# GerHobbelt/ugrep

Hardware: AMD Instinct MI355X
Metric: GB/s scanned + matches/s, 16 GiB synthetic buffer, 1/2/4/8 MI355X (higher is better)
Workload: dtype u8; 1 GPU; 3-literal alternation 'foo|bar|baz' over 16 GiB synthetic ASCII words; config=c2, pattern=foo|bar|baz, bytes_per_gpu=17179869184, total_bytes=17179869184, corpus_kind=1, parallelism=shard1, tables=reference, word=False, dfa_states=9, dfa_row=256, prefilter_ppm=4

## Files before the change

ugrep_amd/csrc/engine.hip:

```cpp
#include <hip/hip_runtime.h>

#include <cstdio>
#include <cstdlib>
#include <cstring>
#include <algorithm>
#include <atomic>
#include <chrono>
#include <condition_variable>
#include <deque>
#include <mutex>
#include <new>
#include <string>
#include <thread>
#include <future>
#include <vector>

#include "../../include/ugpu.h"
#include "plan.hpp"
#include "scan_kernels.hpp"
#include "tables.hpp"

ugpu::Utf8Params utf8_params(const uint8_t* dbuf, uint64_t len)
{
  static std::atomic<int> cached[64];
// ... 154 lines not shown
  static const bool on = std::getenv("UGPU_TRACE") && std::getenv("UGPU_TRACE")[0] == '1';
  return on;
}
#define UGPU_TRACE(...)                  \
  do {                                   \
    if (trace_on()) {                    \
      std::fprintf(stderr, "[ugpu] " __VA_ARGS__); \
      std::fflush(stderr);               \
    }                                    \
  } while (0)

uint64_t env_u64(const char* name, uint64_t dflt)
{
  const char* v = std::getenv(name);
  return v && *v ? std::strtoull(v, nullptr, 0) : dflt;
}

uint32_t acap_lds_n(const ugpu_dfa* d)
{
  if (!d->amode) return 0;
  const size_t n = d->t.ctx_word ? d->t.acap_rows.size() + d->t.states : d->t.acap.size();
  return n <= kSpAcapLds ? (uint32_t)n : 0u;
}

uint32_t fix_rounds_for(const ScanParams& P)
{
  const uint64_t rec = P.tpb * P.unit ? P.tpb * P.unit : 1;
  uint64_t r = env_u64("UGPU_FIX_BUDGET", 256ull << 10) / rec;
  if (r < 4) r = 4;
  if (r > 16) r = 16;
  return (uint32_t)r;
}

int utf8_scan(const uint8_t* dbuf, uint64_t len, bool nul, uint64_t* pos, void* stream);

bool dfa_xc(const ugpu_dfa* d)
{
  const char* env = std::getenv("UGPU_XC");
  return d->t.xc && !d->t.filter && !d->lb && d->t.cap1 != 0 && (!d->d_wtab || d->xcw) && !(env && env[0] == '0');
}

bool dfa_xu(const ugpu_dfa* d)
{
  const char* env = std::getenv("UGPU_XU");
  const bool off = env && env[0] == '0';
  return d->d_xu && (!d->d_wtab || d->wplus) && !off;
}

void fill_tables(ScanParams& P, const ugpu_dfa* d)
{
  P.trans = d->d_trans;
  P.trans32 = d->d_trans32;
  P.xtrans = d->d_xtrans;
  P.xid = d->d_xid;
  P.xid_rows = d->t.xid_rows;
  P.xg = d->d_xg;
  P.xg_sync = d->d_xg_sync;
  P.xg_cls = d->d_xg_sync ? d->d_xg_sync + 256 : nullptr;
  P.xg_stride = 2 * d->t.xg2_pad;
  P.xg_entries = (uint32_t)((d->t.xg2.size() + 7) & ~size_t(7));
  P.cls = d->d_cls;
  P.caps = d->d_caps;
  P.ntrans_pad = d->ntrans_pad;
  P.start = d->t.start;
  P.accb = d->t.accb;
  P.log_row = d->t.log_row;
  P.nstates = d->t.states;
  P.cap1 = d->t.cap1;
  P.wtab = d->d_wtab;
  P.nwtab = d->nwtab;
  P.xc_cls = d->d_cls + 256;
  P.xc_w = d->xcw ? (d->t.xc_w ? 1u : 2u) : 0u;
  P.xu_tab = dfa_xu(d) ? d->d_xu : nullptr;
  P.xu_bm3 = d->d_xu ? reinterpret_cast<const uint32_t*>(d->d_xu + kXuTab) : nullptr;
  P.xu_null = d->t.xu_null;
  P.acap = d->amode ? d->d_acap : nullptr;
  P.ctx_word = d->amode && d->t.ctx_word ? 1u : 0u;
  P.acap_n = (uint32_t)(P.ctx_word ? d->t.acap_rows.size() : d->t.acap.size());
  P.acap_lds = acap_lds_n(d) != 0 && env_u64("UGPU_SP_ACAP_LDS", 1) != 0 ? 1u : 0u;
  P.amap = P.ctx_word ? d->d_acap + d->t.acap_rows.size() : nullptr;
  P.nul = d->nul ? 1u : 0u;
  P.wstart = d->wstart && env_u64("UGPU_WSTART", 1) != 0 ? 1u : 0u;
  P.ft2 = plan_filter2(d->t, d->plan) ? 1u : 0u;
  P.bol0 = 1;
  P.merge_budget = env_u64("UGPU_MERGE_BUDGET", 4096);
  const uint8_t* ft = d->lb ? d->lb_ft : d->t.ft;
  for (int i = 0; i < 5; ++i)
    P.ft[i] = (uint32_t)ft[4 * i] | ((uint32_t)ft[4 * i + 1] << 8) | ((uint32_t)ft[4 * i + 2] << 16) |
              ((uint32_t)ft[4 * i + 3] << 24);
  P.lb_cls = d->lb ? d->d_lbcls : nullptr;
  P.dom = d->d_dom;
  P.look = d->d_look;
  P.dom_all = d->d_dom && d->t.dom_all ? 1u : 0u;
  P.ng_bitmap = d->d_ngram;
  P.ng_n = d->t.ng_n;
  P.ng_log2 = d->t.ng_log2;
  P.ng_tab_lds = d->d_ngram && ngram_tab_lds(d->t.format, d->ntrans_pad, d->nwtab, d->t.ng_log2) ? 1u : 0u;
  if (d->lb) P.wstart = 0;
}

void geometry(ScanParams& P, const uint8_t* dbuf, uint64_t lo, uint64_t hi, uint64_t read_end, int max_rec,
              uint32_t unit, uint32_t per, uint64_t& off)
{
  off = reinterpret_cast<uintptr_t>(dbuf) & 15u;
  P.g = dbuf - off;
  P.lo = lo + off;
  P.hi = hi + off;
  P.rend = read_end + off;
  const uint64_t t0 = P.lo / unit;
  uint64_t t1 = (P.hi + unit - 1) / unit;
  if (t1 <= t0) t1 = t0 + 1;
  const uint64_t nt = t1 - t0;
  uint64_t nrec = nt < (uint64_t)max_rec ? nt : (uint64_t)max_rec;
  if (nrec == 0) nrec = 1;
  const uint64_t min_rec = (nt * unit + kMaxRecBytes - 1) / kMaxRecBytes;
  if (nrec < min_rec) nrec = min_rec < nt ? min_rec : nt;
  const uint64_t tpr = (nt + nrec - 1) / nrec;
  nrec = (nt + tpr - 1) / tpr;
  const uint64_t grid = (nrec + per - 1) / per;
  P.bob = off;
  P.t0 = t0;
  P.t1 = t1;
  P.tpb = tpr;
  P.unit = unit;
  P.grid = (uint32_t)grid;
  P.nrec = (uint32_t)(grid * per);
  P.max_rounds = fix_rounds_for(P);
}

void geometry_for(ScanParams& P, const ugpu_scanner* s, const uint8_t* dbuf, uint64_t lo, uint64_t hi,
                  uint64_t read_end, uint64_t& off, bool xi = false)
{
  if (s->word)
    geometry(P, dbuf, lo, hi, read_end, s->word_rec, wfind_unit(), s->ngram ? ngram_waves() : wfind_waves(), off);
  else if (xi && s->xc)
    geometry(P, dbuf, lo, hi, read_end, s->xi_rec, xc_unit(s->xu), xc_waves(), off);
  else if (xi && s->xg)
    geometry(P, dbuf, lo, hi, read_end, s->xi_rec, xg_unit(), xg_waves(), off);
  else if (xi)
    geometry(P, dbuf, lo, hi, read_end, s->xi_rec, xi_unit(), xi_waves(), off);
  else if (s->sparse)
    geometry(P, dbuf, lo, hi, read_end, s->max_rec, kWaveTile, kSpWaves, off);
  else
    geometry(P, dbuf, lo, hi, read_end, s->max_rec, dense_unit(s->dfa->t.format), dense_waves(s->dfa->t.format), off);
}

hipError_t launch_main(const ugpu_scanner* s, const ScanParams& P, bool write, hipStream_t st, bool xi = false)
{
  if (s->word && s->ngram) return launch_ngram(P, s->dfa->t.format, write, st);
  if (s->word) return launch_wfind(P, s->dfa->t.format, write, st);
  if (xi && s->xc) return launch_xc(P, write, st);
  if (xi && s->xg) return launch_xg(P, st);
  if (xi) return launch_xi(P, s->xi_smem, st);
  if (s->sparse) return launch_sparse(P, write, s->smem, st);
  return launch_dense(P, s->dfa->t.format, write, s->smem, st);
}

bool is_device_ptr(const void* p)
{
  hipPointerAttribute_t a;
  if (hipPointerGetAttributes(&a, p) != hipSuccess) {
    (void)hipGetLastError();
    return false;
  }
  return a.type == hipMemoryTypeDevice;
}
// ... 2803 lines not shown
```

ugrep_amd/csrc/scan_kernels.hpp:

```cpp
#pragma once
#include <hip/hip_runtime.h>
#include <cstdint>

namespace ugpu {

constexpr int kMaxRec = 8192;
constexpr int kFixThreads = 1024;
constexpr int kWaveTile = 4096;
constexpr int kSpWaves = 4;
#ifndef UGPU_DSEG_BYTE
#define UGPU_DSEG_BYTE 188
#endif
#ifndef UGPU_DSEG_CLASS
#define UGPU_DSEG_CLASS 92
#endif
#ifndef UGPU_DWAVES_BYTE
#define UGPU_DWAVES_BYTE 4
#endif
#ifndef UGPU_DWAVES_CLASS
#define UGPU_DWAVES_CLASS 8
#endif
constexpr int kDSegByte = UGPU_DSEG_BYTE;
constexpr int kDSegClass = UGPU_DSEG_CLASS;
constexpr int kDWavesByte = UGPU_DWAVES_BYTE;
// ... 36 lines not shown
};
constexpr uint64_t kOpenConvBudget = 4096;
constexpr uint64_t kOpenSlack = 256;

struct DevTotals {
  uint64_t count, digest, dcap, entry, exit;
  uint32_t flags, rounds;
};

#define UGPU_FLAG_HALO 1u
#define UGPU_FLAG_CAPACITY 2u
#define UGPU_FLAG_BUDGET 4u
#define UGPU_FLAG_WSLOW 32u
#define UGPU_FLAG_NEEDWRITE 64u
#define UGPU_FLAG_USLOW 128u
#define UGPU_FLAG_UMIX 256u
#define UGPU_FLAG_OPEN 512u
constexpr uint32_t kStageOver = 0xffffffffu;
constexpr uint32_t kStageDone = 0xfffffffeu;
constexpr uint32_t kStagePer = 1024;

struct ScanParams {
  const uint8_t* g;
  uint64_t lo, hi;
  uint64_t rend;
  int64_t delta;
  uint32_t at_eof;
  uint32_t ablate;
  uint32_t zero;
  uint64_t t0, t1, tpb;
  uint32_t unit;
  uint32_t nrec;
  uint32_t nstates;
  const uint16_t* trans;
  const uint16_t* xtrans;
  const uint8_t* xid;
  uint32_t xid_rows;
  const uint16_t* xg;
  const uint8_t* xg_sync;
  const uint8_t* xg_cls;
  uint32_t xg_stride;
  uint32_t xg_entries;
  const uint8_t* cls;
  const uint32_t* trans32;
  const uint32_t* caps;
  uint32_t ntrans_pad;
  uint32_t start, accb, log_row;
  uint32_t ft[5];
  uint32_t cap1;
  uint32_t grid;
  BlockRec* recs;
  const uint64_t* entries;
  const uint64_t* out_base;
  uint64_t* out_start;
  uint32_t* out_len;
  uint32_t* out_cap;
  uint64_t out_capacity;
  uint64_t* out_fix;
  uint32_t* flags;
  DevTotals* totals;
  uint64_t* entries_out;
  uint64_t* out_base_out;
  const uint32_t* wtab;
  uint32_t nwtab;
  uint64_t bob;
  uint32_t max_rounds;
  uint64_t merge_budget;
  const uint8_t* xc_cls;
  uint64_t* st_start;
  uint32_t* st_len;
  uint32_t* st_cap;
  uint32_t* st_n;
  uint32_t st_per;
  uint32_t xc_w;
  uint32_t xu_w;
  uint32_t xu_exact;
  const uint8_t* xu_tab;
  const uint32_t* xu_bm3;
  uint32_t xu_null;
  uint16_t* inbits;
  const uint32_t* acap;
  uint32_t wstart;
  uint32_t ft2;
  const uint32_t* lb_cls;
  const uint32_t* dom;
  const uint32_t* look;
  uint32_t dom_all;
  uint32_t bol0;
  uint32_t nul;
  uint32_t ctx_word;
  uint32_t acap_n;
  const uint32_t* amap;
  uint32_t acap_lds;
  OpenRec* open;
  uint32_t* susp;
  SuspRec* srec;
  const uint32_t* ng_bitmap;
  uint32_t ng_n, ng_log2, ng_tab_lds;
};

struct ForestArgs {
  uint64_t c_lo, c_hi;
  uint32_t nblk;
  uint32_t* ex;
  uint64_t* entry;
  uint64_t* run;
  uint64_t* bentry;
  uint64_t* bsum;
  uint64_t* bbase;
};
constexpr uint64_t kFChunk = 64ull << 20;
hipError_t launch_forest(const ScanParams& P, uint32_t format, const ForestArgs& A, uint64_t entry, bool write,
                         DevTotals* tot, hipStream_t stream);
uint64_t forest_block();

hipError_t launch_fix(const ScanParams& P, uint32_t format, hipStream_t stream);
hipError_t launch_pack_records(const uint64_t* start, const uint32_t* len, const uint32_t* cap, uint64_t n,
                               uint64_t base, uint8_t* out, int caps, int dense, uint64_t* esc, uint32_t* nesc,
                               hipStream_t stream);
hipError_t launch_chain_fix(const ScanParams& P, uint32_t format, uint64_t old_entry, uint64_t new_entry,
                            hipStream_t stream);
hipError_t launch_gen(int kind, uint64_t seed, uint64_t off, uint8_t* dbuf, uint64_t len, hipStream_t stream);
hipError_t launch_sparse(const ScanParams& P, bool write, size_t smem, hipStream_t stream);
hipError_t launch_stage_copy(const ScanParams& P, hipStream_t stream);
hipError_t sparse_occupancy(const ScanParams& P, size_t smem, int* blocks_per_cu);
size_t sparse_smem_bytes(uint32_t ntrans_pad, uint32_t nstates, uint32_t nlds_acap = 0);
constexpr uint32_t kSpAcapLds = 2048;
struct LineRec {
  uint64_t first_line, last_line;
  uint64_t trans;
  uint64_t nmatch;
};
struct LinesParams {
  const uint8_t* g;
  uint64_t len;
  uint64_t per;
  uint64_t nwaves;
  const uint64_t* starts;
  uint64_t nmatch;
  uint64_t* counts;
  const uint64_t* prefix;
  uint64_t* lines;
  LineRec* recs;
  uint16_t* qcount;
};
hipError_t launch_nl_count(const LinesParams& L, bool sparse, hipStream_t stream);
hipError_t launch_nl_assign(const LinesParams& L, bool sparse, hipStream_t stream);
uint32_t lines_tile();
constexpr uint32_t kLinesQuarter = 1024;
struct SelParams {
  const uint8_t* g;
  uint64_t len;
  uint64_t per;
  uint64_t nwaves;
  const uint64_t* starts;
  const uint32_t* lens;
  uint64_t nmatch;
  uint32_t invert;
  uint64_t* lastnl;
  uint64_t* mcover;
  const uint64_t* prefix;
  const uint64_t* bol;
  const uint64_t* cover;
  const uint64_t* obase;
  uint64_t* selcnt;
  uint64_t* begin;
// ... 83 lines not shown
```

ugrep_amd/csrc/sparse_kernel.hip:

```cpp
#include "device_common.hpp"

#ifndef UGPU_SP_CTX_OCC
#define UGPU_SP_CTX_OCC 4
#endif
#ifndef UGPU_SP_CTX_WIN
#define UGPU_SP_CTX_WIN 1
#endif

namespace ugpu {

namespace {

struct FTab {
  uint32_t t0lo, t0hi, t1lo, t1hi, t2;
};

template <bool FT2>
__device__ __forceinline__ uint32_t bucket_bits(uint32_t x, const FTab& F)
{
  const uint32_t r0 = __builtin_amdgcn_perm(F.t0hi, F.t0lo, x & 0x07070707u);
  const uint32_t r1 = __builtin_amdgcn_perm(F.t1hi, F.t1lo, (x >> 3) & 0x07070707u);
  if constexpr (FT2) return r0 & r1;
  const uint32_t r2 = __builtin_amdgcn_perm(F.t2, F.t2, (x >> 6) & 0x03030303u);
  return r0 & r1 & r2;
}

__device__ __forceinline__ uint32_t cand_flags(uint32_t R, uint32_t Rn)
{
  return R & __builtin_amdgcn_alignbit(Rn, R, 10) & __builtin_amdgcn_alignbit(Rn, R, 20);
}

__device__ __forceinline__ uint32_t flags4(uint32_t X)
{
  return ((((X | (X >> 1)) & 0x01010101u) * 0x01020408u) >> 24);
}

__device__ __forceinline__ uint32_t letters4(uint32_t x)
{
  const uint32_t t = (x | 0x20202020u) & 0x7f7f7f7fu;
  const uint32_t m = (t + 0x1f1f1f1fu) & ~(t + 0x05050505u) & ~x & 0x80808080u;
  return ((m >> 7) * 0x01020408u) >> 24;
}

__device__ __forceinline__ uint32_t letters16(const uint4& v)
{
  return letters4(v.x) | (letters4(v.y) << 4) | (letters4(v.z) << 8) | (letters4(v.w) << 12);
}

__device__ __forceinline__ uint32_t dpp_scan_add(uint32_t v)
{
  v += __builtin_amdgcn_update_dpp(0, v, 0x111, 0xf, 0xf, false);
  v += __builtin_amdgcn_update_dpp(0, v, 0x112, 0xf, 0xf, false);
  v += __builtin_amdgcn_update_dpp(0, v, 0x114, 0xf, 0xf, false);
  v += __builtin_amdgcn_update_dpp(0, v, 0x118, 0xf, 0xf, false);
  v += __builtin_amdgcn_update_dpp(0, v, 0x142, 0xa, 0xf, false);
  v += __builtin_amdgcn_update_dpp(0, v, 0x143, 0xc, 0xf, false);
  return v;
}

__device__ __forceinline__ uint32_t umax32(uint32_t a, uint32_t b) { return a > b ? a : b; }

__device__ __forceinline__ uint32_t dpp_scan_max(uint32_t v)
{
  v = umax32(v, __builtin_amdgcn_update_dpp(0, v, 0x111, 0xf, 0xf, false));
  v = umax32(v, __builtin_amdgcn_update_dpp(0, v, 0x112, 0xf, 0xf, false));
  v = umax32(v, __builtin_amdgcn_update_dpp(0, v, 0x114, 0xf, 0xf, false));
  v = umax32(v, __builtin_amdgcn_update_dpp(0, v, 0x118, 0xf, 0xf, false));
  v = umax32(v, __builtin_amdgcn_update_dpp(0, v, 0x142, 0xa, 0xf, false));
  v = umax32(v, __builtin_amdgcn_update_dpp(0, v, 0x143, 0xc, 0xf, false));
  return v;
}

__device__ __forceinline__ uint32_t dpp_prev_lane(uint32_t v) { return __builtin_amdgcn_update_dpp(0, v, 0x138, 0xf, 0xf, false); }

__device__ __forceinline__ uint4 load16(const uint8_t* g, uint64_t pos, uint64_t last16)
{
  return *reinterpret_cast<const uint4*>(g + (pos < last16 ? pos : last16));
}

struct TileLoad {
  __amdgpu_buffer_rsrc_t rs;
};

__device__ __forceinline__ uint4 stream16(const TileLoad& L, uint32_t off)
{
  typedef unsigned int v4u __attribute__((ext_vector_type(4)));
  const v4u v = __builtin_amdgcn_raw_buffer_load_b128(L.rs, (int)off, 0, 2 );
  return uint4{v.x, v.y, v.z, v.w};
}

__device__ __forceinline__ void wave_lds_sync()
{
  __builtin_amdgcn_fence(__ATOMIC_RELEASE, "wavefront");
  __builtin_amdgcn_wave_barrier();
  __builtin_amdgcn_fence(__ATOMIC_ACQUIRE, "wavefront");
}

__device__ __forceinline__ uint32_t lanes_below(uint64_t ballot)
{
  return __builtin_amdgcn_mbcnt_hi((uint32_t)(ballot >> 32), __builtin_amdgcn_mbcnt_lo((uint32_t)ballot, 0u));
}

constexpr int kDefer = 64;
constexpr int kAux = 2048;
static_assert(kDefer * 8 <= kAux && 64 * 32 <= kAux, "aux region too small");

struct Stage {
  uint64_t* start = nullptr;
  uint32_t* len = nullptr;
  uint32_t* cap = nullptr;
  uint64_t n = 0;
  uint32_t over = 0;
};

struct WaveChain {
  uint64_t x;
  uint32_t dn;
  uint64_t widx;
  uint32_t wover;
  uint32_t ovf;
  CountEm acc;
  Stage sg;
  uint32_t first, open;
  uint64_t c1, e1;
  uint32_t le1;
  uint32_t pend;
  uint64_t rs, ptile;
  uint64_t wlo;
  uint64_t lbr, lbs;
  uint64_t whi;
};

__device__ __forceinline__ uint64_t readlane64(uint64_t v, int l)
{
  const uint32_t hi = (uint32_t)__builtin_amdgcn_readlane((uint32_t)(v >> 32), l);
  const uint32_t lo = (uint32_t)__builtin_amdgcn_readlane((uint32_t)v, l);
  return ((uint64_t)hi << 32) | lo;
}

template <bool WRITE, bool STAGE = false>
__device__ __forceinline__ void resolve(bool valid, uint64_t c, uint64_t len, uint32_t le, int lane, const Ctx& C,
                                        const ScanParams& P, WaveChain& w)
{
  const uint64_t x = w.x;
  const bool vm = valid && len != 0 && c >= x;
  const uint64_t endr = vm ? c + len - x : 0;
  const bool wide = __ballot(endr > 0xffffffffull) != 0;
  const uint32_t er = (uint32_t)endr, cr = vm ? (uint32_t)(c - x) : 0u;
  const uint32_t pm = dpp_prev_lane(dpp_scan_max(er));
  bool kept = vm && cr >= pm;
  if (wide || __ballot(vm && cr < pm)) {
    uint64_t xx = x;
    kept = false;
    const uint64_t e = vm ? c + len : 0ull;
#pragma unroll 1
    for (int i = 0; i < 64; ++i) {
      const uint64_t ci = __shfl(c, i, 64), ei = __shfl(e, i, 64);
      if (ei != 0 && ci >= xx) {
        if (lane == i) kept = true;
        xx = ei;
      }
    }
  }
  const uint64_t kb = __ballot(kept);
  if (!kb) return;
  const uint64_t rb = __ballot(kept && C.caps[le >> C.log_row] != kCapRedo);
  if constexpr (WRITE) {
    WriteEm we{w.widx + lanes_below(rb), P.out_capacity, P.out_start, P.out_len, P.out_cap};
    if (kept) we.put(C, c, len, le, +1);
    w.wover |= we.overflow;
    w.widx += __popcll(rb);
  } else {
    if (kept) w.acc.put(C, c, len, le, +1);
    if constexpr (STAGE) {
      WriteEm se{w.sg.n + lanes_below(rb), P.st_per, w.sg.start, w.sg.len, w.sg.cap};
      if (kept) se.put(C, c, len, le, +1);
      w.sg.over |= se.overflow;
      w.sg.n += __popcll(rb);
    }
    if (!w.first) {
      const int f = __builtin_ctzll(kb);
      w.first = 1;
      w.c1 = readlane64(c, f);
      w.e1 = w.c1 + readlane64(len, f);
      w.le1 = (uint32_t)__builtin_amdgcn_readlane(le, f);
    }
  }
  w.x = readlane64(c + len, 63 - __builtin_clzll(kb));
// ... 175 lines not shown
    if (s2 > w.x) w.x = s2;
  }
}

template <bool WRITE, bool STAGE>
__device__ __forceinline__ void batch_finish(BatchLane& L, int lane, uint8_t* scr, const Tab<0>& T, const Ctx& C,
                                             const ScanParams& P, WaveChain& w, uint64_t lim, uint64_t gw)
{
  for (;;) {
    const int i = batch_resolve<WRITE, STAGE>(L, lane, C, P, w);
    if (i == 64) break;
    long_lane<WRITE, STAGE>(i, L, lane, scr, T, C, P, w, lim, gw);
    if (w.x == kOpenEnd) break;
  }
  wave_lds_sync();
}

constexpr uint64_t kLbStart = 1ull << 63;
__device__ __forceinline__ bool lb_in(const ScanParams& P, uint32_t b) { return (P.lb_cls[b >> 5] >> (b & 31)) & 1u; }

__device__ __forceinline__ uint64_t lb_back_wave(const ScanParams& P, uint64_t pl, uint64_t bl, int lane)
{
  while (pl > bl) {
    const bool inr = (uint64_t)lane < pl - bl;
    const uint32_t b = inr ? (uint32_t)P.g[pl - 1 - lane] : 0u;
    const uint64_t stop = __ballot(inr && !lb_in(P, b));
    if (stop) return pl - (uint64_t)__builtin_ctzll(stop);
    if (pl - bl <= 64) return bl;
    pl -= 64;
  }
  return pl;
}

__device__ __forceinline__ uint64_t lb_batch(const ScanParams& P, uint64_t e, bool listed, int lane, uint32_t dn,
                                             WaveChain& w)
{
  const bool fixed = listed && (e >> 63) != 0;
  const uint64_t n = listed ? (e & ~kLbStart) : w.lbr;
  const uint32_t plo = (uint32_t)__shfl_up((int)(uint32_t)n, 1, 64);
  const uint32_t phi = (uint32_t)__shfl_up((int)(uint32_t)(n >> 32), 1, 64);
  uint64_t bound = lane == 0 ? w.lbr : (((uint64_t)phi << 32) | plo);
  if (bound < w.wlo) bound = w.wlo;
  if (bound > n) bound = n;
  uint64_t p = n;
  uint32_t steps = 0;
  if (listed && !fixed)
    while (p > bound && steps < 64 && lb_in(P, P.g[p - 1])) {
      --p;
      ++steps;
    }
  const bool longl = listed && !fixed && p > bound && lb_in(P, P.g[p - 1]);
  for (uint64_t lm = __ballot(longl); lm; lm &= lm - 1) {
    const int L = __builtin_ctzll(lm);
    const uint64_t r = lb_back_wave(P, readlane64(p, L), readlane64(bound, L), lane);
    if (lane == L) p = r;
  }
  const bool found = fixed || (listed && p > bound) || (listed && p == bound && bound == w.wlo);
  uint64_t st = found ? p : 0;
#pragma unroll
  for (int d = 1; d < 64; d <<= 1) {
    const uint32_t lo2 = (uint32_t)__shfl_up((int)(uint32_t)st, d, 64);
    const uint32_t hi2 = (uint32_t)__shfl_up((int)(uint32_t)(st >> 32), d, 64);
    const uint64_t o = ((uint64_t)hi2 << 32) | lo2;
    if (lane >= d && o > st) st = o;
  }
  if (w.lbs > st) st = w.lbs;
  const int last = (int)dn - 1;
  w.lbr = readlane64(n, last);
  w.lbs = readlane64(st, last);
  return st;
}

template <bool WRITE, int ABL, int W = kWalkPlain, bool STAGE = false, bool RESUME = false, bool LB = false>
__device__ __forceinline__ void flush_deferred(const uint64_t* dl, uint8_t* scr, uint32_t dn, int lane, const Tab<0>& T,
                                            const Ctx& C, const ScanParams& P, WaveChain& w, uint64_t lim,
                                            uint64_t gw)
{
  wave_lds_sync();
  const bool listed = (uint32_t)lane < dn;
  const uint64_t craw = listed ? dl[lane] : 0;
  bool valid = listed;
  uint64_t c = craw;
  if constexpr (LB) c = lb_batch(P, craw, listed, lane, dn, w);
  const uint64_t a = c & ~uint64_t(15);
  if constexpr (W != kWalkCtx || UGPU_SP_CTX_WIN) {
    const uint64_t last16 = (P.rend - 1) & ~uint64_t(15);
    const uint4 v0 = load16(P.g, a, last16), v1 = load16(P.g, a + 16, last16);
    wave_lds_sync();
    *reinterpret_cast<uint4*>(scr + 32 * lane) = v0;
    *reinterpret_cast<uint4*>(scr + 32 * lane + 16) = v1;
  }
  wave_lds_sync();
  if constexpr (W != kWalkPlain) {
    uint64_t len = 0;
    uint32_t le = 0;
    if (valid && ABL != 3) {
      Win win = win_of(P);
      if constexpr (W == kWalkCtx) {
        if (P.acap_lds) {
          win.acap = C.caps;
          win.amap = C.caps + P.acap_n;
        }
      }
      if constexpr (W == kWalkWord || UGPU_SP_CTX_WIN) {
        win.wl = scr + 32 * lane;
        win.wa = a;
        win.wn = 32;
      }
      len = walk<0, W>(T, win, c, le, w.ovf);
    }
    resolve<WRITE, STAGE>(valid, c, len, le, lane, C, P, w);
    wave_lds_sync();
    return;
  }
  BatchLane L{c, T.start, 0u, 0u, 0u, 0u, valid};
  if (valid && ABL != 3) {
    const uint64_t wl = a + 32 < lim ? a + 32 : lim;
    const uint32_t wr = (uint32_t)(wl - c);
    for (;;) {
      if (L.qr >= wr) {
        if (c + L.qr >= P.rend) {
          if (!P.at_eof) w.ovf = 1;
        } else {
          L.st = c + L.qr >= lim ? 2u : 1u;
        }
        break;
      }
      const uint32_t e = T.step(L.s, scr[32 * lane + (uint32_t)(c - a) + L.qr]);
      if (e == 0) break;
      L.s = e;
      ++L.qr;
      if (e >= T.accb) {
        L.lr = L.qr;
        L.le = e;
      }
    }
  }
  if (!__ballot(L.st != 0)) {
    resolve<WRITE, STAGE>(valid, c, L.lr, L.le, lane, C, P, w);
    wave_lds_sync();
    return;
  }
  wave_lds_sync();
  if constexpr (RESUME) {
    batch_finish<WRITE, STAGE>(L, lane, scr, T, C, P, w, lim, gw);
  } else {
    PendSlot ps;
    ps.c = L.c;
    ps.s = L.s;
    ps.le = L.le;
    ps.packed = L.qr | L.lr << 8 | L.st << 16 | (uint32_t)L.todo << 24;
    ps.pad = 0;
    P.srec[gw].lanes[lane] = ps;
    w.pend = 1;
    w.rs = readlane64(LB ? craw & ~kLbStart : craw, (int)dn - 1) + 1;
  }
}

template <bool WRITE, int ABL, int W = kWalkPlain, bool STAGE = false, bool RESUME = false, bool LB = false,
          bool FT2 = false>
__device__ __forceinline__ void tile_pass(const uint4& v0, const uint4& v1, const uint4& v2, const uint4& v3,
                                          uint64_t ts, bool edge, uint64_t wlo, uint64_t whi, int lane,
                                          const FTab& F, const Tab<0>& T, const Ctx& C, const ScanParams& P,
                                          uint64_t* dl, uint8_t* scr, WaveChain& w, uint64_t lim, uint64_t gw)
{
  if constexpr (ABL == 1) {
    w.acc.cnt += (v0.x ^ v1.y ^ v2.z ^ v3.w) & 1;
    return;
  }
  if (!RESUME && w.pend) return;
  const uint32_t h0 = bucket_bits<FT2>(v0.x, F), h1 = bucket_bits<FT2>(v1.x, F), h2 = bucket_bits<FT2>(v2.x, F),
                 h3 = bucket_bits<FT2>(v3.x, F);
  const uint32_t n0 = __builtin_amdgcn_update_dpp(0, h0, 0x130, 0xf, 0xf, false);
  const uint32_t n1 = __builtin_amdgcn_update_dpp(0, h1, 0x130, 0xf, 0xf, false);
  const uint32_t n2 = __builtin_amdgcn_update_dpp(0, h2, 0x130, 0xf, 0xf, false);
  const uint32_t n3 = __builtin_amdgcn_update_dpp(0, h3, 0x130, 0xf, 0xf, false);
  const uint32_t s1 = __builtin_amdgcn_readlane(h1, 0), s2 = __builtin_amdgcn_readlane(h2, 0),
                 s3 = __builtin_amdgcn_readlane(h3, 0);
  const bool l63 = lane == 63;
  const uint32_t e0 = l63 ? s1 : n0, e1 = l63 ? s2 : n1, e2 = l63 ? s3 : n2, e3 = l63 ? 0x3f3f3f3fu : n3;
  uint32_t X[4][4];
  {
    const uint32_t y = bucket_bits<FT2>(v0.y, F), z = bucket_bits<FT2>(v0.z, F), u = bucket_bits<FT2>(v0.w, F);
    X[0][0] = cand_flags(h0, y);
    X[0][1] = cand_flags(y, z);
    X[0][2] = cand_flags(z, u);
    X[0][3] = cand_flags(u, e0);
  }
  {
    const uint32_t y = bucket_bits<FT2>(v1.y, F), z = bucket_bits<FT2>(v1.z, F), u = bucket_bits<FT2>(v1.w, F);
    X[1][0] = cand_flags(h1, y);
    X[1][1] = cand_flags(y, z);
    X[1][2] = cand_flags(z, u);
    X[1][3] = cand_flags(u, e1);
  }
  {
    const uint32_t y = bucket_bits<FT2>(v2.y, F), z = bucket_bits<FT2>(v2.z, F), u = bucket_bits<FT2>(v2.w, F);
    X[2][0] = cand_flags(h2, y);
    X[2][1] = cand_flags(y, z);
    X[2][2] = cand_flags(z, u);
    X[2][3] = cand_flags(u, e2);
  }
  {
    const uint32_t y = bucket_bits<FT2>(v3.y, F), z = bucket_bits<FT2>(v3.z, F), u = bucket_bits<FT2>(v3.w, F);
    X[3][0] = cand_flags(h3, y);
    X[3][1] = cand_flags(y, z);
    X[3][2] = cand_flags(z, u);
    X[3][3] = cand_flags(u, e3);
  }
  uint32_t lt01 = 0, lt23 = 0;
  if (P.wstart) {
    lt01 = letters16(v0) | (letters16(v1) << 16);
    lt23 = letters16(v2) | (letters16(v3) << 16);
  }
  const uint32_t any0 = X[0][0] | X[0][1] | X[0][2] | X[0][3], any1 = X[1][0] | X[1][1] | X[1][2] | X[1][3];
  const uint32_t any2 = X[2][0] | X[2][1] | X[2][2] | X[2][3], any3 = X[3][0] | X[3][1] | X[3][2] | X[3][3];
  const bool tail = !P.at_eof && ts + kWaveTile + 2 > P.rend && ts < P.rend;
  if (!tail && !__ballot((any0 | any1 | any2 | any3) != 0)) return;
  const uint32_t anyk[4] = {any0, any1, any2, any3};
#pragma unroll
  for (int k = 0; k < 4; ++k) {
    if (!tail && !__ballot(anyk[k] != 0)) continue;
    uint32_t mk = flags4(X[k][0]) | (flags4(X[k][1]) << 4) | (flags4(X[k][2]) << 8) | (flags4(X[k][3]) << 12);
    if (P.wstart) mk &= ~(((k < 2 ? lt01 : lt23) >> (16 * (k & 1))) << 1) & 0xffffu;
    const uint64_t p0 = ts + 1024u * k + 16u * lane;
    if (!P.at_eof && p0 + 18 > P.rend && p0 < P.rend) {
      const uint64_t lo2 = P.rend >= 2 ? P.rend - 2 : 0;
      const uint64_t a = lo2 > p0 ? lo2 - p0 : 0, z = P.rend - p0 > 16 ? 16 : P.rend - p0;
      mk |= (uint32_t)((lowbits(z) & ~lowbits(a)) & 0xffffu);
    }
    if (edge) {
      const uint64_t a = wlo > p0 ? (wlo - p0 > 16 ? 16 : wlo - p0) : 0;
      const uint64_t z = whi > p0 ? (whi - p0 > 16 ? 16 : whi - p0) : 0;
      mk &= (uint32_t)((lowbits(z) & ~lowbits(a)) & 0xffffu);
    }
    const uint64_t xr = w.x > w.rs ? w.x : w.rs;
    if (xr > p0) {
      const uint64_t a = xr - p0;
      mk &= (uint32_t)(~lowbits(a < 16 ? a : 16) & 0xffffu);
    }
    if constexpr (ABL == 2) {
      w.acc.cnt += __popc(mk);
      continue;
    }
    const uint32_t cnt = __popc(mk);
    const uint32_t incl = dpp_scan_add(cnt);
    const uint32_t tot = (uint32_t)__builtin_amdgcn_readlane(incl, 63);
    const uint32_t rank = incl - cnt;
    for (uint32_t done = 0; done < tot;) {
      if (w.dn == (uint32_t)kDefer) {
        flush_deferred<WRITE, ABL, W, STAGE, RESUME, LB>(dl, scr, w.dn, lane, T, C, P, w, lim, gw);
        w.dn = 0;
        if (!RESUME && w.pend) {
          w.ptile = ts;
          return;
        }
      }
      const uint32_t take = tot - done < kDefer - w.dn ? tot - done : kDefer - w.dn;
      uint32_t m = mk, r = rank;
      while (m) {
        const uint32_t bit = __builtin_ctz(m);
        m &= m - 1;
        if (r - done < take) dl[w.dn + r - done] = p0 + bit;
        ++r;
      }
      w.dn += take;
      done += take;
    }
  }
}

__device__ __forceinline__ TileLoad wave_tile(const uint8_t* wbase, uint32_t i, uint32_t rel)
{
  const uint32_t off = i * (uint32_t)kWaveTile;
  const uint32_t n = rel > off ? rel - off : 0u;
  const int nr = __builtin_amdgcn_readfirstlane((int)(n < (uint32_t)kWaveTile ? n : (uint32_t)kWaveTile));
  return TileLoad{__builtin_amdgcn_make_buffer_rsrc(const_cast<uint8_t*>(wbase + off), (short)0, nr, 0x00020000)};
}

}

template <bool WRITE, int ABL, int W = kWalkPlain, bool STAGE = false, bool RESUME = false, bool LB = false,
          bool FT2 = false>
__global__ __launch_bounds__(kSpWaves * 64, RESUME ? 1 : (W == kWalkCtx ? UGPU_SP_CTX_OCC : 6)) void sparse_kernel(ScanParams P)
{
  extern __shared__ __attribute__((aligned(16))) uint8_t smem[];
  const int tid = threadIdx.x, lane = tid & 63;
  const int wid = __builtin_amdgcn_readfirstlane(tid >> 6);
  const uint64_t gw = (uint64_t)blockIdx.x * kSpWaves + wid;
  bool mine = true;
  if constexpr (RESUME) {
    mine = P.susp[gw] != 0;
    if (!__syncthreads_or(mine)) return;
  }
  uint8_t* aux = smem + wid * kAux;
  uint64_t* dl = reinterpret_cast<uint64_t*>(aux);
  uint8_t* scr = aux;
  uint16_t* ltrans = reinterpret_cast<uint16_t*>(smem + kSpWaves * kAux);
  uint32_t* lcaps = reinterpret_cast<uint32_t*>(ltrans + P.ntrans_pad);
  {
    const uint4* src = reinterpret_cast<const uint4*>(P.trans);
    uint4* dst = reinterpret_cast<uint4*>(ltrans);
    for (uint32_t i = tid; i < P.ntrans_pad / 8; i += kSpWaves * 64) dst[i] = src[i];
    for (uint32_t i = tid; i < P.nstates; i += kSpWaves * 64) lcaps[i] = P.caps[i];
    if constexpr (W == kWalkCtx) {
      if (P.acap_lds) {
        uint32_t* la = lcaps + P.nstates;
        for (uint32_t i = tid; i < P.acap_n; i += kSpWaves * 64) la[i] = P.acap[i];
        if (P.ctx_word)
          for (uint32_t i = tid; i < P.nstates; i += kSpWaves * 64) la[P.acap_n + i] = P.amap[i];
      }
    }
  }
  __syncthreads();
  if (!mine) return;
  const Tab<0> T{ltrans, nullptr, P.start, P.accb};
  const Ctx C = W == kWalkCtx ? Ctx{P.acap_lds ? lcaps + P.nstates : P.acap, 0u, P.delta}
                              : Ctx{lcaps, P.log_row, P.delta};
  const FTab F{P.ft[0], P.ft[1], P.ft[2], P.ft[3], P.ft[4]};

  uint64_t tb = P.t0 + gw * P.tpb;
  uint64_t te = tb + P.tpb < P.t1 ? tb + P.tpb : P.t1;
  if (tb > te) tb = te;
  const uint64_t wlo = clampu(tb * kWaveTile, P.lo, P.hi);
  const uint64_t whi = clampu(te * kWaveTile, P.lo, P.hi);
  WaveChain w;
  w.x = WRITE ? P.entries[gw] : wlo;
  w.dn = 0;
  w.widx = WRITE ? P.out_base[gw] : 0;
  w.wover = 0;
  w.ovf = 0;
  w.first = w.open = 0;
  w.c1 = w.e1 = 0;
  w.le1 = 0;
  w.pend = 0;
  w.rs = w.ptile = 0;
  w.wlo = wlo;
  w.whi = whi;
  w.lbr = w.lbs = wlo;
  const uint64_t lim = (W == kWalkPlain && P.open && whi < P.hi) ? whi : P.rend;
  if constexpr (WRITE && !RESUME) {
    if (P.st_n && P.st_n[gw] == kStageDone) {
      if (P.susp && lane == 0) P.susp[gw] = 0;
      return;
    }
  }
  if constexpr (STAGE) {
    w.sg.start = P.st_start + gw * P.st_per;
    w.sg.len = P.st_len + gw * P.st_per;
    w.sg.cap = P.st_cap + gw * P.st_per;
  }

  const uint32_t n = (uint32_t)(te - tb);
  const uint8_t* wbase = P.g + tb * kWaveTile;
  const uint64_t rend16 = (P.rend + 15) & ~uint64_t(15), wb = tb * kWaveTile;
  const uint64_t relw = rend16 > wb ? rend16 - wb : 0;
  const uint32_t rel = (uint32_t)(relw < (uint64_t)n * kWaveTile ? relw : (uint64_t)n * kWaveTile);
  const bool clip_lo = wlo != wb, clip_hi = whi != te * kWaveTile;
  const uint32_t lo16 = 16u * lane;
  uint32_t i = 0;
  if constexpr (RESUME) {
    const SuspRec& sr = P.srec[gw];
    w.x = sr.x;
    w.widx = sr.widx;
    w.wover = sr.wover;
    w.ovf = sr.ovf;
    w.acc.cnt = lane == 0 ? sr.cnt : 0;
    w.acc.dg = lane == 0 ? sr.dg : 0;
    w.acc.dc = lane == 0 ? sr.dc : 0;
    w.sg.n = sr.sgn;
    w.sg.over = sr.sgover;
    w.first = sr.first;
    w.open = sr.open;
    w.c1 = sr.c1;
    w.e1 = sr.e1;
    w.le1 = sr.le1;
    w.rs = sr.rs;
    w.lbr = sr.lbr;
    w.lbs = sr.lbs;
    i = sr.tile;
    const PendSlot ps = sr.lanes[lane];
    BatchLane L{ps.c, ps.s, ps.packed & 0xffu, (ps.packed >> 8) & 0xffu, ps.le, (ps.packed >> 16) & 0xffu,
                (ps.packed >> 24) != 0};
    batch_finish<WRITE, STAGE>(L, lane, scr, T, C, P, w, lim, gw);
  }
  if constexpr (!RESUME && W != kWalkCtx) {
    if (LB && whi > wlo && lb_in(P, P.g[wlo])) {
      if (lane == 0) dl[0] = wlo | kLbStart;
      wave_lds_sync();
      w.dn = 1;
    }
  }
  uint4 a0, a1, a2, a3, b0, b1, b2, b3;
  {
    const TileLoad La = wave_tile(wbase, i, rel);
    a0 = stream16(La, lo16);
    a1 = stream16(La, lo16 + 1024);
    a2 = stream16(La, lo16 + 2048);
    a3 = stream16(La, lo16 + 3072);
    const TileLoad Lb = wave_tile(wbase, i + 1, rel);
    b0 = stream16(Lb, lo16);
    b1 = stream16(Lb, lo16 + 1024);
    b2 = stream16(Lb, lo16 + 2048);
    b3 = stream16(Lb, lo16 + 3072);
  }
  if (n >= i + 2) {
    do {
      tile_pass<WRITE, ABL, W, STAGE, RESUME, LB, FT2>(a0, a1, a2, a3, wb + (uint64_t)i * kWaveTile, i == 0 && clip_lo,
                                                       wlo, whi, lane, F, T, C, P, dl, scr, w, lim, gw);
      {
        const TileLoad L = wave_tile(wbase, i + 2, rel);
        a0 = stream16(L, lo16);
        a1 = stream16(L, lo16 + 1024);
        a2 = stream16(L, lo16 + 2048);
        a3 = stream16(L, lo16 + 3072);
      }
      tile_pass<WRITE, ABL, W, STAGE, RESUME, LB, FT2>(b0, b1, b2, b3, wb + (uint64_t)(i + 1) * kWaveTile,
                                                       i + 2 == n && clip_hi, wlo, whi, lane, F, T, C, P, dl, scr, w,
                                                       lim, gw);
      {
        const TileLoad L = wave_tile(wbase, i + 3, rel);
        b0 = stream16(L, lo16);
        b1 = stream16(L, lo16 + 1024);
        b2 = stream16(L, lo16 + 2048);
        b3 = stream16(L, lo16 + 3072);
      }
      i += 2;
    } while (i + 1 < n);
  }
  if (i < n)
    tile_pass<WRITE, ABL, W, STAGE, RESUME, LB, FT2>(a0, a1, a2, a3, wb + (uint64_t)i * kWaveTile,
                                                     (i == 0 && clip_lo) || clip_hi, wlo, whi, lane, F, T, C, P, dl,
                                                     scr, w, lim, gw);
  if constexpr (LB) {
    if (!w.pend && whi > wlo && lb_in(P, P.g[whi - 1])) {
      const uint64_t r = lb_back_wave(P, whi, wlo, lane);
      {
        if (w.dn == (uint32_t)kDefer) {
          w.ptile = te * kWaveTile;
          flush_deferred<WRITE, ABL, W, STAGE, RESUME, LB>(dl, scr, w.dn, lane, T, C, P, w, lim, gw);
          w.dn = 0;
        }
        if (!w.pend) {
          wave_lds_sync();
          if (lane == 0) dl[w.dn] = r | kLbStart;
          wave_lds_sync();
          ++w.dn;
        }
      }
    }
  }
  if (!w.pend && w.dn) {
    flush_deferred<WRITE, ABL, W, STAGE, RESUME, LB>(dl, scr, w.dn, lane, T, C, P, w, lim, gw);
    w.ptile = te * kWaveTile;
  }
  if constexpr (!RESUME) {
    if (P.susp) {
      if (w.pend) {
        const uint64_t c = wave_sum(w.acc.cnt), d = wave_sum(w.acc.dg), dc = wave_sum(w.acc.dc);
        if (lane == 0) {
          SuspRec* sr = P.srec + gw;
          sr->x = w.x;
          sr->widx = w.widx;
          sr->cnt = c;
          sr->dg = d;
          sr->dc = dc;
          sr->c1 = w.c1;
          sr->e1 = w.e1;
          sr->rs = w.rs;
          sr->lbr = w.lbr;
          sr->lbs = w.lbs;
          sr->sgn = w.sg.n;
          sr->wover = w.wover;
          sr->ovf = w.ovf;
          sr->first = w.first;
          sr->open = w.open;
          sr->le1 = w.le1;
          sr->sgover = w.sg.over;
          sr->tile = (uint32_t)((w.ptile - wb) / kWaveTile);
          sr->dn = 0;
          P.susp[gw] = 1;
        }
        return;
      }
      if (lane == 0) P.susp[gw] = 0;
    }
  }
  uint64_t x = w.x > whi ? w.x : whi;
  if (tb == te) x = wlo;
  if (w.open) x = lim;

  if (w.ovf) atomicOr(P.flags, UGPU_FLAG_HALO);
  if (!WRITE && w.open && lane == 0) atomicOr(P.flags, UGPU_FLAG_OPEN);
  if (w.wover) atomicOr(P.flags, UGPU_FLAG_CAPACITY);
  if constexpr (!WRITE) {
    const uint64_t c = wave_sum(w.acc.cnt), d = wave_sum(w.acc.dg), dc = wave_sum(w.acc.dc);
    if (STAGE && lane == 0) P.st_n[gw] = w.sg.over ? kStageOver : (uint32_t)w.sg.n;
    if (lane == 0) {
      BlockRec rec;
      rec.entry = wlo;
      rec.exit = x;
      rec.cnt = c;
      rec.dg = d;
      rec.dc = dc;
      rec.pad0 = rec.pad1 = rec.pad2 = 0;
      if (W == kWalkPlain) {
        rec.pad0 = w.c1;
        rec.pad1 = w.first ? w.e1 : 0;
// ... 127 lines not shown
```

Before: 6413 GB/s.

## Capture candidate byte windows from registers during sparse scan to skip global reloads

For the plain, non-line-buffered walk, the sparse tile pass now stores each candidate's 32-byte window into a per-slot LDS area straight from the tile registers, taking the next lane's bytes through DPP and readlane. The deferred batch then reloads from global memory only for candidates flagged global, such as the lane-63 edge of the last chunk. It also packs candidate flags with v_lshl_or, uses a ballot-based rank when each lane has at most one candidate, and enlarges the per-wave aux LDS region. The aim is to remove scattered global reloads and a wave sync per deferred batch, at the cost of extra LDS per wave (lower occupancy risk) and more register shuffling on candidate tiles.

```diff
diff --git a/ugrep_amd/csrc/engine.hip b/ugrep_amd/csrc/engine.hip
--- a/ugrep_amd/csrc/engine.hip
+++ b/ugrep_amd/csrc/engine.hip
@@ -260,6 +260,7 @@
   P.nul = d->nul ? 1u : 0u;
   P.wstart = d->wstart && env_u64("UGPU_WSTART", 1) != 0 ? 1u : 0u;
   P.ft2 = plan_filter2(d->t, d->plan) ? 1u : 0u;
+  P.sp_win = env_u64("UGPU_SP_WIN", 1) != 0 ? 1u : 0u;
   P.bol0 = 1;
   P.merge_budget = env_u64("UGPU_MERGE_BUDGET", 4096);
   const uint8_t* ft = d->lb ? d->lb_ft : d->t.ft;
diff --git a/ugrep_amd/csrc/scan_kernels.hpp b/ugrep_amd/csrc/scan_kernels.hpp
--- a/ugrep_amd/csrc/scan_kernels.hpp
+++ b/ugrep_amd/csrc/scan_kernels.hpp
@@ -142,6 +142,7 @@
   const uint32_t* acap;
   uint32_t wstart;
   uint32_t ft2;
+  uint32_t sp_win;
   const uint32_t* lb_cls;
   const uint32_t* dom;
   const uint32_t* look;
diff --git a/ugrep_amd/csrc/sparse_kernel.hip b/ugrep_amd/csrc/sparse_kernel.hip
--- a/ugrep_amd/csrc/sparse_kernel.hip
+++ b/ugrep_amd/csrc/sparse_kernel.hip
@@ -28,6 +28,14 @@
 __device__ __forceinline__ uint32_t cand_flags(uint32_t R, uint32_t Rn)
 {
   return R & __builtin_amdgcn_alignbit(Rn, R, 10) & __builtin_amdgcn_alignbit(Rn, R, 20);
+}
+
+__device__ __forceinline__ uint32_t pack_flags(const uint32_t (&X)[4])
+{
+  const uint32_t lo = X[0] | (X[1] << 2), hi = X[2] | (X[3] << 2);
+  uint32_t r;
+  asm("v_lshl_or_b32 %0, %1, 4, %2" : "=v"(r) : "v"(hi), "v"(lo));
+  return r;
 }
 
 __device__ __forceinline__ uint32_t flags4(uint32_t X)
@@ -102,8 +110,12 @@
 }
 
 constexpr int kDefer = 64;
-constexpr int kAux = 2048;
-static_assert(kDefer * 8 <= kAux && 64 * 32 <= kAux, "aux region too small");
+constexpr int kList = kDefer * 8;
+constexpr int kAux = kList + kDefer * 32;
+static_assert(kAux % 16 == 0 && kList % 16 == 0 && 64 * 16 <= kDefer * 32, "aux region layout");
+constexpr uint64_t kWinGlobal = 1ull << 62;
+template <int W, bool LB>
+constexpr bool capture_windows = W == kWalkPlain && !LB;
 
 struct Stage {
   uint64_t* start = nullptr;
@@ -445,15 +457,27 @@
   bool valid = listed;
   uint64_t c = craw;
   if constexpr (LB) c = lb_batch(P, craw, listed, lane, dn, w);
+  if constexpr (capture_windows<W, LB>) c = craw & ~kWinGlobal;
   const uint64_t a = c & ~uint64_t(15);
-  if constexpr (W != kWalkCtx || UGPU_SP_CTX_WIN) {
+  if constexpr (capture_windows<W, LB>) {
+    const bool glob = listed && (craw & kWinGlobal) != 0;
+    if (__ballot(glob)) {
+      if (glob) {
+        const uint64_t last16 = (P.rend - 1) & ~uint64_t(15);
+        const uint4 v0 = load16(P.g, a, last16), v1 = load16(P.g, a + 16, last16);
+        *reinterpret_cast<uint4*>(scr + 32 * lane) = v0;
+        *reinterpret_cast<uint4*>(scr + 32 * lane + 16) = v1;
+      }
+      wave_lds_sync();
+    }
+  } else if constexpr (W != kWalkCtx || UGPU_SP_CTX_WIN) {
     const uint64_t last16 = (P.rend - 1) & ~uint64_t(15);
     const uint4 v0 = load16(P.g, a, last16), v1 = load16(P.g, a + 16, last16);
     wave_lds_sync();
     *reinterpret_cast<uint4*>(scr + 32 * lane) = v0;
     *reinterpret_cast<uint4*>(scr + 32 * lane + 16) = v1;
   }
-  wave_lds_sync();
+  if constexpr (!capture_windows<W, LB>) wave_lds_sync();
   if constexpr (W != kWalkPlain) {
     uint64_t len = 0;
     uint32_t le = 0;
@@ -516,7 +540,7 @@
     ps.pad = 0;
     P.srec[gw].lanes[lane] = ps;
     w.pend = 1;
-    w.rs = readlane64(LB ? craw & ~kLbStart : craw, (int)dn - 1) + 1;
+    w.rs = readlane64(LB ? craw & ~kLbStart : c, (int)dn - 1) + 1;
   }
 }
 
@@ -572,22 +596,41 @@
     X[3][3] = cand_flags(u, e3);
   }
   uint32_t lt01 = 0, lt23 = 0;
-  if (P.wstart) {
+  if (!capture_windows<W, LB> && P.wstart) {
     lt01 = letters16(v0) | (letters16(v1) << 16);
     lt23 = letters16(v2) | (letters16(v3) << 16);
   }
-  const uint32_t any0 = X[0][0] | X[0][1] | X[0][2] | X[0][3], any1 = X[1][0] | X[1][1] | X[1][2] | X[1][3];
-  const uint32_t any2 = X[2][0] | X[2][1] | X[2][2] | X[2][3], any3 = X[3][0] | X[3][1] | X[3][2] | X[3][3];
+  constexpr bool CAP = capture_windows<W, LB>;
+  uint32_t any0, any1, any2, any3;
+  if constexpr (CAP) {
+    any0 = pack_flags(X[0]);
+    any1 = pack_flags(X[1]);
+    any2 = pack_flags(X[2]);
+    any3 = pack_flags(X[3]);
+  } else {
+    any0 = X[0][0] | X[0][1] | X[0][2] | X[0][3], any1 = X[1][0] | X[1][1] | X[1][2] | X[1][3];
+    any2 = X[2][0] | X[2][1] | X[2][2] | X[2][3], any3 = X[3][0] | X[3][1] | X[3][2] | X[3][3];
+  }
   const bool tail = !P.at_eof && ts + kWaveTile + 2 > P.rend && ts < P.rend;
   if (!tail && !__ballot((any0 | any1 | any2 | any3) != 0)) return;
   const uint32_t anyk[4] = {any0, any1, any2, any3};
 #pragma unroll
   for (int k = 0; k < 4; ++k) {
     if (!tail && !__ballot(anyk[k] != 0)) continue;
-    uint32_t mk = flags4(X[k][0]) | (flags4(X[k][1]) << 4) | (flags4(X[k][2]) << 8) | (flags4(X[k][3]) << 12);
-    if (P.wstart) mk &= ~(((k < 2 ? lt01 : lt23) >> (16 * (k & 1))) << 1) & 0xffffu;
+    uint32_t mk;
+    if constexpr (CAP)
+      mk = flags4(anyk[k]) | (flags4(anyk[k] >> 2) << 4) | (flags4(anyk[k] >> 4) << 8) |
+           (flags4(anyk[k] >> 6) << 12);
+    else
+      mk = flags4(X[k][0]) | (flags4(X[k][1]) << 4) | (flags4(X[k][2]) << 8) | (flags4(X[k][3]) << 12);
+    if constexpr (CAP) {
+      if (P.wstart) mk &= ~(letters16(k == 0 ? v0 : k == 1 ? v1 : k == 2 ? v2 : v3) << 1) & 0xffffu;
+    } else {
+      if (P.wstart) mk &= ~(((k < 2 ? lt01 : lt23) >> (16 * (k & 1))) << 1) & 0xffffu;
+    }
+    const uint64_t cs = ts + 1024u * k;
     const uint64_t p0 = ts + 1024u * k + 16u * lane;
-    if (!P.at_eof && p0 + 18 > P.rend && p0 < P.rend) {
+    if ((CAP ? tail : !P.at_eof) && p0 + 18 > P.rend && p0 < P.rend) {
       const uint64_t lo2 = P.rend >= 2 ? P.rend - 2 : 0;
       const uint64_t a = lo2 > p0 ? lo2 - p0 : 0, z = P.rend - p0 > 16 ? 16 : P.rend - p0;
       mk |= (uint32_t)((lowbits(z) & ~lowbits(a)) & 0xffffu);
@@ -598,7 +641,7 @@
       mk &= (uint32_t)((lowbits(z) & ~lowbits(a)) & 0xffffu);
     }
     const uint64_t xr = w.x > w.rs ? w.x : w.rs;
-    if (xr > p0) {
+    if ((!CAP || xr > cs) && xr > p0) {
       const uint64_t a = xr - p0;
       mk &= (uint32_t)(~lowbits(a < 16 ? a : 16) & 0xffffu);
     }
@@ -607,9 +650,16 @@
       continue;
     }
     const uint32_t cnt = __popc(mk);
-    const uint32_t incl = dpp_scan_add(cnt);
-    const uint32_t tot = (uint32_t)__builtin_amdgcn_readlane(incl, 63);
-    const uint32_t rank = incl - cnt;
+    uint32_t rank, tot;
+    if (CAP && !__ballot(cnt > 1)) {
+      const uint64_t hb = __ballot(mk != 0);
+      rank = lanes_below(hb);
+      tot = (uint32_t)__popcll(hb);
+    } else {
+      const uint32_t incl = dpp_scan_add(cnt);
+      tot = (uint32_t)__builtin_amdgcn_readlane(incl, 63);
+      rank = incl - cnt;
+    }
     for (uint32_t done = 0; done < tot;) {
       if (w.dn == (uint32_t)kDefer) {
         flush_deferred<WRITE, ABL, W, STAGE, RESUME, LB>(dl, scr, w.dn, lane, T, C, P, w, lim, gw);
@@ -620,17 +670,54 @@
         }
       }
       const uint32_t take = tot - done < kDefer - w.dn ? tot - done : kDefer - w.dn;
+      const uint4& vc = k == 0 ? v0 : k == 1 ? v1 : k == 2 ? v2 : v3;
+      uint4 nx{0u, 0u, 0u, 0u};
+      bool glob = false;
+      if constexpr (CAP) {
+        glob = !P.sp_win || (k == 3 && l63);
+        if (P.sp_win) {
+          nx.x = __builtin_amdgcn_update_dpp(0, vc.x, 0x130, 0xf, 0xf, false);
+          nx.y = __builtin_amdgcn_update_dpp(0, vc.y, 0x130, 0xf, 0xf, false);
+          nx.z = __builtin_amdgcn_update_dpp(0, vc.z, 0x130, 0xf, 0xf, false);
+          nx.w = __builtin_amdgcn_update_dpp(0, vc.w, 0x130, 0xf, 0xf, false);
+          if (k < 3) {
+            const uint4& vn = k == 0 ? v1 : k == 1 ? v2 : v3;
+            const uint32_t sx = __builtin_amdgcn_readlane(vn.x, 0), sy = __builtin_amdgcn_readlane(vn.y, 0),
+                           sz = __builtin_amdgcn_readlane(vn.z, 0), sw = __builtin_amdgcn_readlane(vn.w, 0);
+            if (l63) nx = uint4{sx, sy, sz, sw};
+          }
+        }
+      }
       uint32_t m = mk, r = rank;
       while (m) {
         const uint32_t bit = __builtin_ctz(m);
         m &= m - 1;
-        if (r - done < take) dl[w.dn + r - done] = p0 + bit;
+        if (r - done < take) {
+          const uint32_t slot = w.dn + r - done;
+          dl[slot] = CAP ? (p0 + bit) | (glob ? kWinGlobal : 0ull) : p0 + bit;
+          if constexpr (CAP) {
+            if (!glob) {
+              *reinterpret_cast<uint4*>(scr + 32 * slot) = vc;
+              *reinterpret_cast<uint4*>(scr + 32 * slot + 16) = nx;
+            }
+          }
+        }
         ++r;
       }
       w.dn += take;
       done += take;
     }
   }
+}
+
+template <bool IMM>
+__device__ __forceinline__ void load_tile(const TileLoad& L, uint32_t lo16, uint4& r0, uint4& r1, uint4& r2, uint4& r3)
+{
+  if constexpr (IMM) asm volatile("" : "+v"(lo16));
+  r0 = stream16(L, lo16);
+  r1 = stream16(L, lo16 + 1024);
+  r2 = stream16(L, lo16 + 2048);
+  r3 = stream16(L, lo16 + 3072);
 }
 
 __device__ __forceinline__ TileLoad wave_tile(const uint8_t* wbase, uint32_t i, uint32_t rel)
@@ -658,7 +745,7 @@
   }
   uint8_t* aux = smem + wid * kAux;
   uint64_t* dl = reinterpret_cast<uint64_t*>(aux);
-  uint8_t* scr = aux;
+  uint8_t* scr = aux + (capture_windows<W, LB> ? kList : 0);
   uint16_t* ltrans = reinterpret_cast<uint16_t*>(smem + kSpWaves * kAux);
   uint32_t* lcaps = reinterpret_cast<uint32_t*>(ltrans + P.ntrans_pad);
   {
@@ -757,15 +844,9 @@
   uint4 a0, a1, a2, a3, b0, b1, b2, b3;
   {
     const TileLoad La = wave_tile(wbase, i, rel);
-    a0 = stream16(La, lo16);
-    a1 = stream16(La, lo16 + 1024);
-    a2 = stream16(La, lo16 + 2048);
-    a3 = stream16(La, lo16 + 3072);
+    load_tile<capture_windows<W, LB>>(La, lo16, a0, a1, a2, a3);
     const TileLoad Lb = wave_tile(wbase, i + 1, rel);
-    b0 = stream16(Lb, lo16);
-    b1 = stream16(Lb, lo16 + 1024);
-    b2 = stream16(Lb, lo16 + 2048);
-    b3 = stream16(Lb, lo16 + 3072);
+    load_tile<capture_windows<W, LB>>(Lb, lo16, b0, b1, b2, b3);
   }
   if (n >= i + 2) {
     do {
@@ -773,20 +854,14 @@
                                                        wlo, whi, lane, F, T, C, P, dl, scr, w, lim, gw);
       {
         const TileLoad L = wave_tile(wbase, i + 2, rel);
-        a0 = stream16(L, lo16);
-        a1 = stream16(L, lo16 + 1024);
-        a2 = stream16(L, lo16 + 2048);
-        a3 = stream16(L, lo16 + 3072);
+        load_tile<capture_windows<W, LB>>(L, lo16, a0, a1, a2, a3);
       }
       tile_pass<WRITE, ABL, W, STAGE, RESUME, LB, FT2>(b0, b1, b2, b3, wb + (uint64_t)(i + 1) * kWaveTile,
                                                        i + 2 == n && clip_hi, wlo, whi, lane, F, T, C, P, dl, scr, w,
                                                        lim, gw);
       {
         const TileLoad L = wave_tile(wbase, i + 3, rel);
-        b0 = stream16(L, lo16);
-        b1 = stream16(L, lo16 + 1024);
-        b2 = stream16(L, lo16 + 2048);
-        b3 = stream16(L, lo16 + 3072);
+        load_tile<capture_windows<W, LB>>(L, lo16, b0, b1, b2, b3);
       }
       i += 2;
     } while (i + 1 < n);
```

Result: no change. 6366 GB/s (-0.7%).
